# micahvista/VACmap

Hardware: AMD Instinct MI355X
Metric: aligned Gbp/s (whole node) + reads/s, 15 kb ONT-shape reads vs hg38-size ref, 1/2/4/8 MI355X (higher is better)
Workload: dtype i16/i32 DP + f64 chains

## Files before the change

### vacmap_amd/csrc/k_dp.hip

```cpp
#include "vmx_device.h"
#include "vmx_kernels.h"

__device__ __forceinline__ int vmx_tcode(uint8_t c) { return c < 4 ? (int)c : 6; }


__global__ void k_encode(const char* __restrict__ in, uint8_t* __restrict__ out, int64_t n) {
    int64_t i = (int64_t)blockIdx.x * blockDim.x + threadIdx.x;
    int64_t stride = (int64_t)gridDim.x * blockDim.x;
    for (; i < n; i += stride) out[i] = vmx_code((uint8_t)in[i]);
}

#define VMX_EXT_RING 512
__global__ void __launch_bounds__(64) k_extend(const uint8_t* __restrict__ tcodes, const int64_t* __restrict__ t_off,
                                               const uint8_t* __restrict__ qcodes, const int64_t* __restrict__ q_off, int n_prob,
                                               int match, int mismatch, int o, int e, int bw_in, int zdrop,
                                               int32_t* __restrict__ out_te, int32_t* __restrict__ out_qe, int32_t* __restrict__ out_sc, const int32_t* __restrict__ n_ptr) {
    if (n_ptr) n_prob = *n_ptr;
    __shared__ int sH[3][VMX_EXT_RING];
    __shared__ int sE[2][VMX_EXT_RING];
    __shared__ int sF[2][VMX_EXT_RING];
    const int lane = vmx_lane();
    const int RM = VMX_EXT_RING - 1;
    for (int p = blockIdx.x; p < n_prob; p += gridDim.x) {
        const uint8_t* T = tcodes + t_off[p];
// ... 331 lines not shown
                    const int j63 = t - 62;                                         \
                    if (j63 >= 1 && j63 <= ql && ((j63 & 63) == 0 || j63 == ql)) {                                    \
                        const int col = j63 - lane;                      \
                        if (col > ((j63 - 1) & ~63)) { bH[col] = sH; bE1[col] = sE1; bE2[col] = sE2; }                \
                    }                                                                                                 \
                }                                                                                                     \
            }
            for (int t0 = 0; t0 < W; t0 += 64) {
                const int jj = t0 + lane;
                int qchunk = jj < ql ? (int)Q[jj] : 4;
                int cH = 0, cE1 = VMX_NEG, cE2 = VMX_NEG;
                if (jj + 1 <= ql) {
                    if (s == 0) cH = vmx_gap_open_row(jj + 1, o1, e1, o2, e2);
                    else { cH = bH[jj + 1]; cE1 = bE1[jj + 1]; cE2 = bE2[jj + 1]; }
                }
                if (t0 >= 64 && t0 + 64 <= ql) {
                    for (int tt = 0; tt < 64; ++tt) { const int t = t0 + tt; VMX_GF_STEP(true) }
                } else {
                    int tend = W - t0; if (tend > 64) tend = 64;
                    for (int tt = 0; tt < tend; ++tt) { const int t = t0 + tt; const int j = t - lane + 1; VMX_GF_STEP(j >= 1 && j <= ql) }
                }
            }
#undef VMX_GF_STEP
            __syncthreads();
        }
        if (!trivial && !pk && lane == ((tl - 1) & 63)) out_score[p] = outH;
        int32_t sink = 0;
        if (pk) vmx_gapfill_fill16(T, Q, tl, ql, match, mismatch, o1, e1, o2, e2, tb, bH, SCORE ? &out_score[p] : &sink, lane);
}

template <bool SCORE>
__device__ __forceinline__ void vmx_gapfill_fill_body(const uint8_t* __restrict__ tcodes, const uint8_t* __restrict__ qcodes,
                                                     const vmx_dp_prob* __restrict__ probs, int n_prob, int match, int mismatch,
                                                     int o1, int e1, int o2, int e2, uint8_t* __restrict__ tb_pool,
                                                     int32_t* __restrict__ bnd_pool, int32_t* __restrict__ out_score,
                                                     const int32_t* __restrict__ order, int32_t* __restrict__ counter,
                                                     int32_t* __restrict__ redo_list = nullptr, int32_t* __restrict__ redo_cnt = nullptr, int redo_pass = 0,
                                                     uint8_t* __restrict__ redo_pool = nullptr) {
    const int lane = vmx_lane();
    int static_next = 4 * (int)blockIdx.x;
    if (redo_pass) {
        n_prob = redo_cnt[0]; order = redo_list; counter = redo_cnt + 1;
        while (true) {
            int q; { int v = 0; if (lane == 0) v = atomicAdd(redo_cnt + 2, 1); q = vmx_bcast0(v); }
            if (q >= n_prob) break;
            const int p = order[q];
            const int tl = probs[p].tl, ql = probs[p].ql;
            if (VMX_REDO_PK(tl, ql)) vmx_gapfill_fill_one<SCORE>(tcodes, qcodes, probs, p, match, mismatch, o1, e1, o2, e2, tb_pool, bnd_pool, out_score, lane, VMX_PK_FLAG, redo_pool);
        }
    }
    while (true) {
        int q0;
        if (order) { int v = 0; if (lane == 0) v = atomicAdd(counter, 4); q0 = vmx_bcast0(v); }
        else { q0 = static_next; static_next += 4 * (int)gridDim.x; }
        if (q0 >= n_prob) break;
        const int qg = q0 + (lane >> 4);
        const int pg = qg < n_prob ? (order ? order[qg] : qg) : -1;
        bool x4 = false, skip = false;
        {
            vmx_dp_prob pr; pr.tl = 0; pr.ql = 0; pr.t_off = 0; pr.q_off = 0; pr.tb_off = 0; pr.bnd_off = 0;
            if (pg >= 0) pr = probs[pg];
            skip = redo_pass && pg >= 0 && VMX_REDO_PK(pr.tl, pr.ql);
            x4 = pg >= 0 && !skip && pr.tl > 0 && pr.ql > 0 && VMX_DP16X4_OK(pr.tl, pr.ql);
            if (!SCORE && x4 && (lane & 15) == 0) out_score[pg] = 0;
            if (__any(x4))
                vmx_gapfill_fill16x4<SCORE>(tcodes + pr.t_off, qcodes + pr.q_off, x4 ? pr.tl : 0, x4 ? pr.ql : 0, match, mismatch, o1, e1, o2, e2, vmx_tb_ptr(tb_pool, redo_pool, pr.tb_off),
                                            bnd_pool + pr.bnd_off, &out_score[pg < 0 ? 0 : pg], lane);
        }
        for (int gk = 0; gk < 4; ++gk) {
            const int p = vmx_readlane(pg, 16 * gk);
            if (p < 0 || vmx_readlane((int)(x4 || skip), 16 * gk)) continue;
            vmx_gapfill_fill_one<SCORE>(tcodes, qcodes, probs, p, match, mismatch, o1, e1, o2, e2, tb_pool, bnd_pool, out_score, lane, 0, redo_pool);
        }
    }
}

__device__ __forceinline__ void vmx_gapfill_ad_pass(const uint8_t* __restrict__ tcodes, const uint8_t* __restrict__ qcodes, vmx_dp_prob* __restrict__ probs, int n_prob,
                                                   int match, int mismatch, int o1, int e1, int o2, int e2, uint8_t* __restrict__ tb_pool, int32_t* __restrict__ bnd_pool,
                                                   int32_t* __restrict__ out_score, const int32_t* __restrict__ order, const int32_t* __restrict__ range, int32_t* __restrict__ counter,
                                                   int32_t* __restrict__ redo_list, int32_t* __restrict__ redo_cnt, int ad_pct, unsigned long long* __restrict__ redo_bytes,
                                                   unsigned long long redo_cap, int tb_by_ns) {
    const int lane = vmx_lane();
    const int pct = ad_pct & 0xffff, pct_min = (ad_pct >> 16) & 0xffff;
    const int n_head = range[0] < n_prob ? range[0] : n_prob;
    bool head = n_head > 0;
    while (true) {
        int pX = -1, pY = -1;
        if (head) {
            int q; { int v = 0; if (lane == 0) v = atomicAdd(counter + 1, 1); q = vmx_bcast0(v); }
            if (q >= n_head) { head = false; continue; }
            if (lane < 16) pX = order[q];
        } else {
            int q0; { int v = 0; if (lane == 0) v = atomicAdd(counter, 8); q0 = n_head + vmx_bcast0(v); }
            if (q0 >= n_prob) break;
            const int qX = q0 + 2 * (lane >> 4), qY = qX + 1;
            if (qX < n_prob) pX = order[qX];
            if (qY < n_prob) pY = order[qY];
        }
        vmx_dp_prob prX, prY;
        prX.tl = 0; prX.ql = 0; prX.t_off = 0; prX.q_off = 0; prX.tb_off = 0; prY = prX;
        if (pX >= 0) prX = probs[pX];
        if (pY >= 0) prY = probs[pY];
        const bool x4X = pX >= 0 && prX.tl > 0 && prX.ql > 0 && VMX_DP16X4_OK(prX.tl, prX.ql), x4Y = pY >= 0 && prY.tl > 0 && prY.ql > 0 && VMX_DP16X4_OK(prY.tl, prY.ql);
        const int nsX = x4X ? vmx_ad_ns(prX.tl, prX.ql, match, o1, e1, o2, e2, pct, pct_min) : 0, nsY = x4Y ? vmx_ad_ns(prY.tl, prY.ql, match, o1, e1, o2, e2, pct, pct_min) : 0;
        const int ns = vmx_uniform_i32(vmx_wave_max_i32(nsX > nsY ? nsX : nsY));
        bool keepX = false, keepY = false, triedX = false, triedY = false;
        if (ns > 0) {
            int dloX = 0, dloY = 0;
            const bool fitX = !tb_by_ns || VMX_AD_W(nsX) == VMX_AD_W(ns), fitY = !tb_by_ns || VMX_AD_W(nsY) == VMX_AD_W(ns);
            const int gX = (nsX > 0 && fitX) ? vmx_ad_geom(prX.tl, prX.ql, ns, &dloX) : 0, gY = (nsY > 0 && fitY) ? vmx_ad_geom(prY.tl, prY.ql, ns, &dloY) : 0;
            const int tlX = gX > 0 ? prX.tl : 0, qlX = gX > 0 ? prX.ql : 0, tlY = gY > 0 ? prY.tl : 0, qlY = gY > 0 ? prY.ql : 0;
            int scX = 0, scY = 0;
#define VMX_AD_RUN(NSV) vmx_gapfill_fill_ad<NSV>(tcodes + prX.t_off, qcodes + prX.q_off, tlX, qlX, dloX, tb_pool + prX.tb_off, tcodes + prY.t_off, qcodes + prY.q_off, tlY, qlY, dloY, \
                                                 tb_pool + prY.tb_off, match, mismatch, o1, e1, o2, e2, lane, scX, scY)
            if (ns == 1) VMX_AD_RUN(1); else if (ns == 2) VMX_AD_RUN(2); else if (ns == 3) VMX_AD_RUN(3); else VMX_AD_RUN(4);
#undef VMX_AD_RUN
            triedX = gX > 0; triedY = gY > 0;
            keepX = gX > 0 && vmx_ad_proven(scX, prX.tl, prX.ql, gX, match, o1, e1, o2, e2);
            keepY = gY > 0 && vmx_ad_proven(scY, prY.tl, prY.ql, gY, match, o1, e1, o2, e2);
        }
        if ((lane & 15) == 0) {
            if (x4X) {
                out_score[pX] = keepX ? VMX_AD_FLAG + ns : 0;
                if (!keepX) {
                    if (triedX) atomicAdd(redo_cnt + 3, 1);
                    const unsigned long long need = (unsigned long long)VMX_REDO_TB_BYTES(prX.tl, prX.ql), at = atomicAdd(redo_bytes, need);
                    if (at + need > redo_cap) { probs[pX].tl = 0; probs[pX].ql = 0; probs[pX].tb_off = 0; }
                    else { probs[pX].tb_off = -(int64_t)at - 1; redo_list[atomicAdd(redo_cnt, 1)] = pX; }
                }
            }
            if (x4Y) {
                out_score[pY] = keepY ? VMX_AD_FLAG + ns : 0;
                if (!keepY) {
                    if (triedY) atomicAdd(redo_cnt + 3, 1);
                    const unsigned long long need = (unsigned long long)VMX_REDO_TB_BYTES(prY.tl, prY.ql), at = atomicAdd(redo_bytes, need);
                    if (at + need > redo_cap) { probs[pY].tl = 0; probs[pY].ql = 0; probs[pY].tb_off = 0; }
                    else { probs[pY].tb_off = -(int64_t)at - 1; redo_list[atomicAdd(redo_cnt, 1)] = pY; }
                }
            }
        }
        for (int gk = 0; gk < 8; ++gk) {
            const int p = vmx_readlane((gk & 1) ? pY : pX, 16 * (gk >> 1));
            if (p < 0 || vmx_readlane((int)((gk & 1) ? x4Y : x4X), 16 * (gk >> 1))) continue;
            vmx_gapfill_fill_one<false>(tcodes, qcodes, probs, p, match, mismatch, o1, e1, o2, e2, tb_pool, bnd_pool, out_score, lane);
        }
    }
}

__global__ void __launch_bounds__(64) k_gapfill_fill(const uint8_t* __restrict__ tcodes, const uint8_t* __restrict__ qcodes,
                                                     const vmx_dp_prob* __restrict__ probs, int n_prob, int match, int mismatch,
                                                     int o1, int e1, int o2, int e2, uint8_t* __restrict__ tb_pool,
                                                     int32_t* __restrict__ bnd_pool, int32_t* __restrict__ out_score,
                                                     const int32_t* __restrict__ order, int32_t* __restrict__ counter) {
    vmx_gapfill_fill_body<true>(tcodes, qcodes, probs, n_prob, match, mismatch, o1, e1, o2, e2, tb_pool, bnd_pool, out_score, order, counter);
}
__global__ void __launch_bounds__(64, 4) k_gapfill_fill_ns(const uint8_t* __restrict__ tcodes, const uint8_t* __restrict__ qcodes,
                                                        vmx_dp_prob* __restrict__ probs, int n_prob, int match, int mismatch,
                                                        int o1, int e1, int o2, int e2, uint8_t* __restrict__ tb_pool,
                                                        int32_t* __restrict__ bnd_pool, int32_t* __restrict__ out_score,
                                                        const int32_t* __restrict__ order, const int32_t* __restrict__ range, int32_t* __restrict__ counter,
                                                        int32_t* __restrict__ redo_list, int32_t* __restrict__ redo_cnt, int redo_pass, int ad_pct,
                                                        uint8_t* __restrict__ redo_pool, unsigned long long* __restrict__ redo_bytes, const int32_t* __restrict__ n_ptr,
                                                        unsigned long long redo_cap, int tb_by_ns) {
    if (n_ptr) n_prob = *n_ptr;
    if (redo_pass) vmx_gapfill_fill_body<false>(tcodes, qcodes, probs, n_prob, match, mismatch, o1, e1, o2, e2, tb_pool, bnd_pool, out_score, order, counter, redo_list, redo_cnt, 1, redo_pool);
    else vmx_gapfill_ad_pass(tcodes, qcodes, probs, n_prob, match, mismatch, o1, e1, o2, e2, tb_pool, bnd_pool, out_score, order, range, counter, redo_list, redo_cnt, ad_pct, redo_bytes, redo_cap, tb_by_ns);
}

__global__ void k_gapfill_trace(const uint8_t* __restrict__ tcodes, const uint8_t* __restrict__ qcodes,
                                const vmx_dp_prob* __restrict__ probs, int n_prob, int eqx, const uint8_t* __restrict__ tb_pool,
                                uint32_t* __restrict__ run_pool, char* __restrict__ cig_pool, int32_t* __restrict__ cig_len,
                                const int32_t* __restrict__ band_flag, const uint8_t* __restrict__ redo_pool, int spread, int32_t* __restrict__ cig_q,
                                const int32_t* __restrict__ n_ptr) {
    VMX_SETPRIO(3);
    if (n_ptr) n_prob = *n_ptr;
    const int gt = (int)(blockIdx.x * blockDim.x + threadIdx.x);
    if (spread > 1 && gt % spread) return;
    int p = spread > 1 ? gt / spread : gt;
    if (p >= n_prob) return;
    const vmx_dp_prob pr = probs[p];
    const uint8_t* T = tcodes + pr.t_off;
    const uint8_t* Q = qcodes + pr.q_off;
    const int tl = pr.tl, ql = pr.ql;
    const uint8_t* tb = vmx_tb_ptr(tb_pool, redo_pool, pr.tb_off);
    uint32_t* runs = run_pool + pr.run_off;
    char* cig = cig_pool + pr.cig_off;
    bool x4 = tl > 0 && ql > 0 && VMX_DP16X4_OK(tl, ql);
// ... 75 lines not shown
```

### vacmap_amd/csrc/vmx_device.h

```cpp
#ifndef VMX_DEVICE_H
#define VMX_DEVICE_H
#ifdef VMX_EMU
#include "hip_emu.h"
#define VMX_DYN_SHARED(type, name) type* name = (type*)hipemu::cur()->dynshared
#else
#include <hip/hip_runtime.h>
#define VMX_DYN_SHARED(type, name) extern __shared__ __attribute__((aligned(16))) type name[]
#endif
#include <stdint.h>

#define VMX_WAVE 64
#define VMX_NEG (-(1 << 28))
#define VMX_NOPRE (-9999999)

__device__ __forceinline__ int vmx_lane() { return (int)(threadIdx.x & 63); }

#ifdef VMX_EMU
__device__ __forceinline__ int vmx_shr1(int v) { return __shfl_up(v, 1); }
__device__ __forceinline__ int vmx_readlane(int v, int l) { return __shfl(v, l); }
#define VMX_SPIN_PAUSE() hipemu::yield()
#define VMX_CLOCK() 0LL
#else
__device__ __forceinline__ int vmx_shr1(int v) { return __builtin_amdgcn_update_dpp(v, v, 0x138, 0xf, 0xf, false); }
__device__ __forceinline__ int vmx_readlane(int v, int l) { return __builtin_amdgcn_readlane(v, l); }
#define VMX_SPIN_PAUSE() __builtin_amdgcn_s_sleep(1)
#define VMX_CLOCK() ((long long)wall_clock64())
#endif
#ifdef VMX_EMU
__device__ __forceinline__ int vmx_shr1_in(int v, int in) { int e = __shfl_up(v, 1); return vmx_lane() == 0 ? in : e; }
__device__ __forceinline__ int vmx_rol1(int v) { return __shfl(v, (vmx_lane() + 1) & 63); }
__device__ __forceinline__ int vmx_ror1(int v) { return __shfl(v, (vmx_lane() + 63) & 63); }
#else
__device__ __forceinline__ int vmx_shr1_in(int v, int in) { return __builtin_amdgcn_update_dpp(in, v, 0x138, 0xf, 0xf, false); }
__device__ __forceinline__ int vmx_rol1(int v) { return __builtin_amdgcn_update_dpp(v, v, 0x134, 0xf, 0xf, false); }
__device__ __forceinline__ int vmx_ror1(int v) { return __builtin_amdgcn_update_dpp(v, v, 0x13C, 0xf, 0xf, false); }
#endif
#ifdef VMX_EMU
__device__ __forceinline__ unsigned vmx_pk(int lo, int hi) { return ((unsigned)lo & 0xffffu) | ((unsigned)hi << 16); }
__device__ __forceinline__ int vmx_pk_lo(unsigned a) { return (int)(short)(a & 0xffffu); }
__device__ __forceinline__ int vmx_pk_hi(unsigned a) { return (int)(short)(a >> 16); }
__device__ __forceinline__ unsigned vmx_pk_add(unsigned a, unsigned b) { return vmx_pk(vmx_pk_lo(a) + vmx_pk_lo(b), vmx_pk_hi(a) + vmx_pk_hi(b)); }
__device__ __forceinline__ unsigned vmx_pk_sub(unsigned a, unsigned b) { return vmx_pk(vmx_pk_lo(a) - vmx_pk_lo(b), vmx_pk_hi(a) - vmx_pk_hi(b)); }
__device__ __forceinline__ unsigned vmx_pk_max(unsigned a, unsigned b) {
    const int l = vmx_pk_lo(a) > vmx_pk_lo(b) ? vmx_pk_lo(a) : vmx_pk_lo(b), h = vmx_pk_hi(a) > vmx_pk_hi(b) ? vmx_pk_hi(a) : vmx_pk_hi(b);
    return vmx_pk(l, h);
}
__device__ __forceinline__ unsigned vmx_pk_neg(unsigned a) { return (vmx_pk_lo(a) < 0 ? 0xffffu : 0u) | (vmx_pk_hi(a) < 0 ? 0xffff0000u : 0u); }
__device__ __forceinline__ unsigned vmx_pk_min_u16(unsigned a, unsigned b) { const unsigned al = a & 0xffffu, bl = b & 0xffffu, ah = a >> 16, bh = b >> 16; return (al < bl ? al : bl) | ((ah < bh ? ah : bh) << 16); }
__device__ __forceinline__ unsigned vmx_pk_mad(unsigned a, unsigned b, unsigned c) { return vmx_pk(vmx_pk_lo(a) * vmx_pk_lo(b) + vmx_pk_lo(c), vmx_pk_hi(a) * vmx_pk_hi(b) + vmx_pk_hi(c)); }
__device__ __forceinline__ unsigned vmx_alignbit16(unsigned hi, unsigned lo) { return (hi << 16) | (lo >> 16); }
#else
typedef short vmx_v2s __attribute__((ext_vector_type(2)));
__device__ __forceinline__ unsigned vmx_pk(int lo, int hi) { return ((unsigned)lo & 0xffffu) | ((unsigned)hi << 16); }
__device__ __forceinline__ int vmx_pk_lo(unsigned a) { return (int)(short)(a & 0xffffu); }
__device__ __forceinline__ int vmx_pk_hi(unsigned a) { return (int)(short)(a >> 16); }
__device__ __forceinline__ unsigned vmx_pk_add(unsigned a, unsigned b) { return __builtin_bit_cast(unsigned, (vmx_v2s)(__builtin_bit_cast(vmx_v2s, a) + __builtin_bit_cast(vmx_v2s, b))); }
__device__ __forceinline__ unsigned vmx_pk_sub(unsigned a, unsigned b) { return __builtin_bit_cast(unsigned, (vmx_v2s)(__builtin_bit_cast(vmx_v2s, a) - __builtin_bit_cast(vmx_v2s, b))); }
__device__ __forceinline__ unsigned vmx_pk_max(unsigned a, unsigned b) { return __builtin_bit_cast(unsigned, __builtin_elementwise_max(__builtin_bit_cast(vmx_v2s, a), __builtin_bit_cast(vmx_v2s, b))); }
__device__ __forceinline__ unsigned vmx_pk_neg(unsigned a) { unsigned r; asm("v_pk_ashrrev_i16 %0, 15, %1 op_sel_hi:[0,1]" : "=v"(r) : "v"(a)); return r; }
__device__ __forceinline__ unsigned vmx_pk_min_u16(unsigned a, unsigned b) { unsigned r; asm("v_pk_min_u16 %0, %1, %2" : "=v"(r) : "v"(a), "v"(b)); return r; }
__device__ __forceinline__ unsigned vmx_pk_mad(unsigned a, unsigned b, unsigned c) { unsigned r; asm("v_pk_mad_i16 %0, %1, %2, %3" : "=v"(r) : "v"(a), "v"(b), "v"(c)); return r; }
__device__ __forceinline__ unsigned vmx_alignbit16(unsigned hi, unsigned lo) { return __builtin_amdgcn_alignbit(hi, lo, 16); }
#endif
#ifdef VMX_EMU
__device__ __forceinline__ unsigned vmx_pk_bytes(unsigned b) { return (b & 0xffu) | ((b >> 8) & 0xff00u); }
#else
__device__ __forceinline__ unsigned vmx_pk_bytes(unsigned b) { return __builtin_amdgcn_perm(b, b, 0x0c0c0200u); }
#endif
#if defined(VMX_EMU) || defined(VMX_NOPRIO)
#define VMX_SETPRIO(p) ((void)0)
#else
#define VMX_SETPRIO(p) __builtin_amdgcn_s_setprio(p)
#endif
#ifdef VMX_EMU
__device__ __forceinline__ void vmx_wave_lds_fence() { __syncthreads(); }
#else
__device__ __forceinline__ void vmx_wave_lds_fence() { asm volatile("" ::: "memory"); }
#endif
__device__ __forceinline__ unsigned vmx_bfi(unsigned m, unsigned a, unsigned b) { return (m & a) | (~m & b); }
#ifdef VMX_EMU
__device__ __forceinline__ int vmx_uniform_i32(int v) { return v; }
#else
__device__ __forceinline__ int vmx_uniform_i32(int v) { return __builtin_amdgcn_readfirstlane(v); }
#endif
__device__ __forceinline__ long long vmx_uniform_i64(long long v) {
    union { long long d; int i[2]; } u; u.d = v;
    u.i[0] = vmx_uniform_i32(u.i[0]); u.i[1] = vmx_uniform_i32(u.i[1]);
    return u.d;
}
__device__ __forceinline__ double vmx_uniform_f64(double v) {
    union { double d; int i[2]; } u; u.d = v;
    u.i[0] = vmx_uniform_i32(u.i[0]); u.i[1] = vmx_uniform_i32(u.i[1]);
    return u.d;
}
#ifdef VMX_EMU
#define VMX_GLOBAL_PTR(T, p) (p)
#else
#define VMX_GLOBAL_PTR(T, p) ((T*)(__attribute__((address_space(1))) T*)(unsigned long long)vmx_uniform_i64((long long)(p)))
#endif
#ifdef VMX_EMU
__device__ __forceinline__ int vmx_bcast0(int v) { return __shfl(v, 0); }
#else
__device__ __forceinline__ int vmx_bcast0(int v) { return __builtin_amdgcn_readfirstlane(v); }
#endif
__device__ __forceinline__ double vmx_shr1_f64(double v) {
    union { double d; int i[2]; } u; u.d = v;
    u.i[0] = vmx_shr1(u.i[0]); u.i[1] = vmx_shr1(u.i[1]);
    return u.d;
}
__device__ __forceinline__ long long vmx_shr1_i64(long long v) {
    union { long long d; int i[2]; } u; u.d = v;
    u.i[0] = vmx_shr1(u.i[0]); u.i[1] = vmx_shr1(u.i[1]);
    return u.d;
}
struct vmx_cwin { int j, q, ls; double S; long long r; };
__device__ __forceinline__ void vmx_cwin_insert(vmx_cwin& w, int at, int k, double Sk, int qk, int lsk, long long rk, int lane) {
    const int sj = vmx_shr1(w.j), sq = vmx_shr1(w.q), sls = vmx_shr1(w.ls);
    const double sS = vmx_shr1_f64(w.S); const long long sr = vmx_shr1_i64(w.r);
    if (lane > at) { w.j = sj; w.q = sq; w.ls = sls; w.S = sS; w.r = sr; }
    else if (lane == at) { w.j = k; w.q = qk; w.ls = lsk; w.S = Sk; w.r = rk; }
}
__device__ __forceinline__ double vmx_readlane_f64(double v, int l) {
    union { double d; int i[2]; } u; u.d = v;
    u.i[0] = vmx_readlane(u.i[0], l); u.i[1] = vmx_readlane(u.i[1], l);
    return u.d;
}

__device__ __forceinline__ int vmx_wave_max_i32(int v) {
    for (int o = 32; o > 0; o >>= 1) { int x = __shfl_xor(v, o); v = x > v ? x : v; }
    return v;
}
__device__ __forceinline__ int vmx_wave_sum_i32(int v) {
    for (int o = 32; o > 0; o >>= 1) v += __shfl_xor(v, o);
    return v;
}
__device__ __forceinline__ long long vmx_wave_sum_i64(long long v) {
    for (int o = 32; o > 0; o >>= 1) v += __shfl_xor(v, o);
    return v;
}
__device__ __forceinline__ int vmx_wave_incl_scan_i32(int v) {
    int lane = vmx_lane();
    for (int o = 1; o < 64; o <<= 1) { int x = __shfl_up(v, o); if (lane >= o) v += x; }
    return v;
// ... 350 lines not shown
```

### vacmap_amd/csrc/vmx_dp_ad.h

```cpp
#ifndef VMX_DP_AD_H
#define VMX_DP_AD_H

#ifdef VMX_EMU
__device__ __forceinline__ int vmx_r16_shl1_in(int v, int in) { const int l = vmx_lane(); const int e = __shfl(v, (l & 48) | ((l + 1) & 15)); return (l & 15) == 15 ? in : e; }
__device__ __forceinline__ unsigned vmx_perm(unsigned s0, unsigned s1, unsigned sel) {
    unsigned r = 0;
    for (int b = 0; b < 4; ++b) {
        const unsigned c = (sel >> (8 * b)) & 0xffu;
        const unsigned v = c < 4 ? (s1 >> (8 * c)) & 0xffu : c < 8 ? (s0 >> (8 * (c - 4))) & 0xffu : 0u;
        r |= v << (8 * b);
    }
    return r;
}
#else
__device__ __forceinline__ int vmx_r16_shl1_in(int v, int in) { return __builtin_amdgcn_update_dpp(in, v, 0x101, 0xf, 0xf, false); }
__device__ __forceinline__ unsigned vmx_perm(unsigned s0, unsigned s1, unsigned sel) { return __builtin_amdgcn_perm(s0, s1, sel); }
#endif

#define VMX_AD_BIAS 8192
#define VMX_AD_NEGINF (-4096)
struct vmx_ad_consts { unsigned O1, O2, E1, E2, MATCH, NMIS, ONE, NEGP; };

__device__ __forceinline__ unsigned vmx_ad_cell(const vmx_ad_consts& K, unsigned upH, unsigned upE1, unsigned upE2, unsigned leftH, unsigned leftF1,
                                                unsigned leftF2, unsigned tc, unsigned qc, unsigned& H, unsigned& E1, unsigned& E2, unsigned& F1, unsigned& F2) {
    const unsigned a1 = upH - K.O1, a2 = upH - K.O2;
    unsigned b = (unsigned)((int)vmx_pk_sub(a1, upE1) >> 12) & 0x00080008u;
    b |= (unsigned)((int)vmx_pk_sub(a2, upE2) >> 11) & 0x00100010u;
    const unsigned e1v = vmx_pk_max(a1, upE1) - K.E1, e2v = vmx_pk_max(a2, upE2) - K.E2;
    const unsigned c1 = leftH - K.O1, c2 = leftH - K.O2;
    b |= (unsigned)((int)vmx_pk_sub(c1, leftF1) >> 10) & 0x00200020u;
    b |= (unsigned)((int)vmx_pk_sub(c2, leftF2) >> 9) & 0x00400040u;
    const unsigned f1v = vmx_pk_max(c1, leftF1) - K.E1, f2v = vmx_pk_max(c2, leftF2) - K.E2;
    unsigned h = vmx_pk_mad(vmx_pk_min_u16(tc ^ qc, K.ONE), K.NMIS, H) + K.MATCH;
    unsigned src = 0, m;
    m = vmx_pk_neg(vmx_pk_sub(h, e1v)); src = vmx_bfi(m, 0x00010001u, src); h = vmx_pk_max(h, e1v);
    m = vmx_pk_neg(vmx_pk_sub(h, f1v)); src = vmx_bfi(m, 0x00030003u, src); h = vmx_pk_max(h, f1v);
    m = vmx_pk_neg(vmx_pk_sub(h, e2v)); src = vmx_bfi(m, 0x00020002u, src); h = vmx_pk_max(h, e2v);
    m = vmx_pk_neg(vmx_pk_sub(h, f2v)); src = vmx_bfi(m, 0x00040004u, src); h = vmx_pk_max(h, f2v);
    H = h; E1 = e1v; E2 = e2v; F1 = f1v; F2 = f2v;
    return b | src;
}

template <int NS>
__device__ __forceinline__ unsigned vmx_ad_pick(const unsigned (&v)[NS], int k) {
    unsigned r = 0;
#pragma unroll
    for (int i = 0; i < NS; ++i) r |= v[i] & (unsigned)-(int)(k == i);
    return r;
}

template <int NS>
__device__ __forceinline__ void vmx_gapfill_fill_ad(const uint8_t* __restrict__ TX, const uint8_t* __restrict__ QX, int tlX, int qlX, int dloX, uint8_t* __restrict__ tbX,
                                                   const uint8_t* __restrict__ TY, const uint8_t* __restrict__ QY, int tlY, int qlY, int dloY, uint8_t* __restrict__ tbY,
                                                   int match, int mismatch, int o1, int e1, int o2, int e2, int lane, int& scoreX, int& scoreY) {
    const int l = lane & 15;
    vmx_ad_consts K;
    K.O1 = vmx_pk(o1, o1); K.O2 = vmx_pk(o2, o2); K.E1 = vmx_pk(e1, e1); K.E2 = vmx_pk(e2, e2);
    K.MATCH = vmx_pk(match, match); K.NMIS = vmx_pk(mismatch - match, mismatch - match); K.ONE = vmx_pk(1, 1); K.NEGP = vmx_pk(VMX_AD_NEGINF + VMX_AD_BIAS, VMX_AD_NEGINF + VMX_AD_BIAS);
    const int afX = (tlX > 0 && qlX > 0) ? tlX + qlX : 0, afY = (tlY > 0 && qlY > 0) ? tlY + qlY : 0;
    const int total = vmx_uniform_i32(vmx_wave_max_i32(afX > afY ? afX : afY));
    const int npairs = (total + 1) >> 1;
    const int poX = (afX + 1) >> 1, peX = afX >> 1, poY = (afY + 1) >> 1, peY = afY >> 1;
    const int hX = dloX >> 1, hY = dloY >> 1;
    auto tcf = [&](const uint8_t* T, int tl, int i) -> int { return (i >= 1 && i <= tl) ? vmx_tcode(T[i - 1]) : 5; };
    auto qcf = [&](const uint8_t* Q, int ql, int j) -> int { return (j >= 1 && j <= ql) ? (int)Q[j - 1] : 4; };
    unsigned tcode[NS], qcode[NS];
#pragma unroll
    for (int k = 0; k < NS; ++k) {
        tcode[k] = vmx_pk(tcf(TX, tlX, -hX - NS * l - k), tcf(TY, tlY, -hY - NS * l - k));
        qcode[k] = vmx_pk(qcf(QX, qlX, hX + NS * l + k), qcf(QY, qlY, hY + NS * l + k));
    }
    unsigned HA[NS], E1A[NS], E2A[NS], F1A[NS], F2A[NS], HC[NS], E1C[NS], E2C[NS], F1C[NS], F2C[NS];
    {
        const int l0X = (-dloX) / (2 * NS), k0X = ((-dloX) % (2 * NS)) >> 1, l0Y = (-dloY) / (2 * NS), k0Y = ((-dloY) % (2 * NS)) >> 1;
#pragma unroll
        for (int k = 0; k < NS; ++k) {
            const unsigned m = ((l == l0X && k == k0X) ? 0xffffu : 0u) | ((l == l0Y && k == k0Y) ? 0xffff0000u : 0u);
            HA[k] = vmx_bfi(m, vmx_pk(VMX_AD_BIAS, VMX_AD_BIAS), K.NEGP);
            E1A[k] = K.NEGP; E2A[k] = K.NEGP; F1A[k] = K.NEGP; F2A[k] = K.NEGP;
            HC[k] = K.NEGP; E1C[k] = K.NEGP; E2C[k] = K.NEGP; F1C[k] = K.NEGP; F2C[k] = K.NEGP;
        }
    }
    const int xfX = (qlX - tlX) - dloX, xfY = (qlY - tlY) - dloY;
    const int lfX = xfX / (2 * NS), kfX = (xfX % (2 * NS)) >> 1, lfY = xfY / (2 * NS), kfY = (xfY % (2 * NS)) >> 1;
    int finX = 0, finY = 0;
    constexpr int W = VMX_AD_W(NS);
    uint8_t* const pX = tbX + VMX_AD_TB_OFF_W(0, l, W);
    uint8_t* const pY = tbY + VMX_AD_TB_OFF_W(0, l, W);
    auto put = [&](uint8_t* at, unsigned w01, unsigned w23, bool hi) {
        if constexpr (W == 1) *at = (uint8_t)(hi ? (w01 >> 16) : w01);
        else if constexpr (W == 2) *(uint16_t*)at = (uint16_t)(hi ? (w01 >> 16) : w01);
        else *(uint32_t*)at = vmx_perm(w23, w01, hi ? 0x07060302u : 0x05040100u);
    };
    auto load_chunks = [&](int b16, unsigned& tch, unsigned& qch) {
        tch = vmx_pk(tcf(TX, tlX, b16 + 1 + l - hX), tcf(TY, tlY, b16 + 1 + l - hY));
        qch = vmx_pk(qcf(QX, qlX, b16 + 15 - l + hX + 16 * NS), qcf(QY, qlY, b16 + 15 - l + hY + 16 * NS));
    };
    unsigned tch, qch, ntch, nqch;
    load_chunks(0, ntch, nqch);
    for (int p0 = 0; p0 < npairs; p0 += 16) {
        tch = ntch; qch = nqch;
        load_chunks(p0 + 16, ntch, nqch);
        int pend = npairs - p0; if (pend > 16) pend = 16;
        for (int pp = 0; pp < pend; ++pp) {
            const int p = p0 + pp + 1;
            {
                const unsigned in = (unsigned)vmx_r16_shl1_in((int)qcode[0], (int)qch);
#pragma unroll
                for (int k = 0; k + 1 < NS; ++k) qcode[k] = qcode[k + 1];
                qcode[NS - 1] = in;
                qch = (unsigned)vmx_r16_ror1((int)qch);
            }
            unsigned bb[NS];
            {
                const unsigned nH = (unsigned)vmx_r16_shl1_in((int)HA[0], (int)K.NEGP), nE1 = (unsigned)vmx_r16_shl1_in((int)E1A[0], (int)K.NEGP),
                               nE2 = (unsigned)vmx_r16_shl1_in((int)E2A[0], (int)K.NEGP);
#pragma unroll
                for (int k = 0; k < NS; ++k) {
                    const unsigned uH = k + 1 < NS ? HA[k + 1 < NS ? k + 1 : 0] : nH, uE1 = k + 1 < NS ? E1A[k + 1 < NS ? k + 1 : 0] : nE1, uE2 = k + 1 < NS ? E2A[k + 1 < NS ? k + 1 : 0] : nE2;
                    bb[k] = vmx_ad_cell(K, uH, uE1, uE2, HA[k], F1A[k], F2A[k], tcode[k], qcode[k], HC[k], E1C[k], E2C[k], F1C[k], F2C[k]);
                }
            }
            {
                unsigned w01 = bb[0], w23 = 0;
                if (NS > 1) w01 |= bb[NS > 1 ? 1 : 0] << 8;
                if (NS > 2) w23 = bb[NS > 2 ? 2 : 0];
                if (NS > 3) w23 |= bb[NS > 3 ? 3 : 0] << 8;
                const size_t so = VMX_AD_TB_OFF_W(2 * p - 2, 0, W);
                if (p <= poX) put(pX + so, w01, w23, false);
                if (p <= poY) put(pY + so, w01, w23, true);
            }
            {
                const unsigned in = (unsigned)vmx_r16_shr1_in((int)tcode[NS - 1], (int)tch);
#pragma unroll
                for (int k = NS - 1; k > 0; --k) tcode[k] = tcode[k - 1];
                tcode[0] = in;
                tch = (unsigned)vmx_r16_rol1((int)tch);
            }
            {
                const unsigned nH = (unsigned)vmx_r16_shr1_in((int)HC[NS - 1], (int)K.NEGP), nF1 = (unsigned)vmx_r16_shr1_in((int)F1C[NS - 1], (int)K.NEGP),
                               nF2 = (unsigned)vmx_r16_shr1_in((int)F2C[NS - 1], (int)K.NEGP);
#pragma unroll
                for (int k = 0; k < NS; ++k) {
                    const unsigned lH = k > 0 ? HC[k > 0 ? k - 1 : 0] : nH, lF1 = k > 0 ? F1C[k > 0 ? k - 1 : 0] : nF1, lF2 = k > 0 ? F2C[k > 0 ? k - 1 : 0] : nF2;
                    bb[k] = vmx_ad_cell(K, HC[k], E1C[k], E2C[k], lH, lF1, lF2, tcode[k], qcode[k], HA[k], E1A[k], E2A[k], F1A[k], F2A[k]);
                }
            }
            {
                unsigned w01 = bb[0], w23 = 0;
                if (NS > 1) w01 |= bb[NS > 1 ? 1 : 0] << 8;
                if (NS > 2) w23 = bb[NS > 2 ? 2 : 0];
                if (NS > 3) w23 |= bb[NS > 3 ? 3 : 0] << 8;
                const size_t so = VMX_AD_TB_OFF_W(2 * p - 1, 0, W);
                if (p <= peX) put(pX + so, w01, w23, false);
                if (p <= peY) put(pY + so, w01, w23, true);
            }
            if (__any(p == poX || p == poY)) {
                const unsigned aX = vmx_ad_pick<NS>(HA, kfX), cX = vmx_ad_pick<NS>(HC, kfX), aY = vmx_ad_pick<NS>(HA, kfY), cY = vmx_ad_pick<NS>(HC, kfY);
                const unsigned vX = (afX & 1) ? cX : aX, vY = (afY & 1) ? cY : aY;
                if (p == poX && l == lfX) finX = vmx_pk_lo(vX) - VMX_AD_BIAS;
                if (p == poY && l == lfY) finY = vmx_pk_hi(vY) - VMX_AD_BIAS;
            }
        }
    }
    scoreX = __shfl(finX, (lane & 48) | (lfX & 15));
    scoreY = __shfl(finY, (lane & 48) | (lfY & 15));
}

__device__ __forceinline__ bool vmx_ad_proven(int score, int tl, int ql, int g, int match, int o1, int e1, int o2, int e2) {
    const int mn = tl < ql ? tl : ql;
    if (g < 1) return false;
    if (g > mn) return true;
    const long long U = (long long)match * mn - vmx_ad_margin(g, match, o1, e1, o2, e2);
    return (long long)score > U;
}
#endif
```

Baseline: 3.168.

## Tag traceback source in low bits of scaled unsigned 16-bit DP scores

Reworks the anti-diagonal 16x4 gap-fill cell so scores are scaled by 8 and biased into unsigned 16-bit lanes, with the low 3 bits carrying a source tag. The max operations then yield the traceback source directly, replacing the per-cell compare/negate/bfi chain. Traceback bytes are packed once per pair of cells via byte permutes. The aim is fewer VALU instructions per cell in the hot DP loop. In exchange it narrows the usable score range, so a host/device check now disables the AD path for scoring schemes that do not fit.

Measured after the change: 3.375, median of 6. 1.07x the previous value.

```diff
diff --git a/vacmap_amd/csrc/k_dp.hip b/vacmap_amd/csrc/k_dp.hip
--- a/vacmap_amd/csrc/k_dp.hip
+++ b/vacmap_amd/csrc/k_dp.hip
@@ -437,6 +437,7 @@
                                                    unsigned long long redo_cap, int tb_by_ns) {
     const int lane = vmx_lane();
     const int pct = ad_pct & 0xffff, pct_min = (ad_pct >> 16) & 0xffff;
+    const bool ad_ok = vmx_ad_scores_ok(match, mismatch, o1, e1, o2, e2);
     const int n_head = range[0] < n_prob ? range[0] : n_prob;
     bool head = n_head > 0;
     while (true) {
@@ -457,7 +458,7 @@
         if (pX >= 0) prX = probs[pX];
         if (pY >= 0) prY = probs[pY];
         const bool x4X = pX >= 0 && prX.tl > 0 && prX.ql > 0 && VMX_DP16X4_OK(prX.tl, prX.ql), x4Y = pY >= 0 && prY.tl > 0 && prY.ql > 0 && VMX_DP16X4_OK(prY.tl, prY.ql);
-        const int nsX = x4X ? vmx_ad_ns(prX.tl, prX.ql, match, o1, e1, o2, e2, pct, pct_min) : 0, nsY = x4Y ? vmx_ad_ns(prY.tl, prY.ql, match, o1, e1, o2, e2, pct, pct_min) : 0;
+        const int nsX = x4X && ad_ok ? vmx_ad_ns(prX.tl, prX.ql, match, o1, e1, o2, e2, pct, pct_min) : 0, nsY = x4Y && ad_ok ? vmx_ad_ns(prY.tl, prY.ql, match, o1, e1, o2, e2, pct, pct_min) : 0;
         const int ns = vmx_uniform_i32(vmx_wave_max_i32(nsX > nsY ? nsX : nsY));
         bool keepX = false, keepY = false, triedX = false, triedY = false;
         if (ns > 0) {
diff --git a/vacmap_amd/csrc/vmx_device.h b/vacmap_amd/csrc/vmx_device.h
--- a/vacmap_amd/csrc/vmx_device.h
+++ b/vacmap_amd/csrc/vmx_device.h
@@ -47,6 +47,7 @@
 }
 __device__ __forceinline__ unsigned vmx_pk_neg(unsigned a) { return (vmx_pk_lo(a) < 0 ? 0xffffu : 0u) | (vmx_pk_hi(a) < 0 ? 0xffff0000u : 0u); }
 __device__ __forceinline__ unsigned vmx_pk_min_u16(unsigned a, unsigned b) { const unsigned al = a & 0xffffu, bl = b & 0xffffu, ah = a >> 16, bh = b >> 16; return (al < bl ? al : bl) | ((ah < bh ? ah : bh) << 16); }
+__device__ __forceinline__ unsigned vmx_pk_max_u16(unsigned a, unsigned b) { const unsigned al = a & 0xffffu, bl = b & 0xffffu, ah = a >> 16, bh = b >> 16; return (al > bl ? al : bl) | ((ah > bh ? ah : bh) << 16); }
 __device__ __forceinline__ unsigned vmx_pk_mad(unsigned a, unsigned b, unsigned c) { return vmx_pk(vmx_pk_lo(a) * vmx_pk_lo(b) + vmx_pk_lo(c), vmx_pk_hi(a) * vmx_pk_hi(b) + vmx_pk_hi(c)); }
 __device__ __forceinline__ unsigned vmx_alignbit16(unsigned hi, unsigned lo) { return (hi << 16) | (lo >> 16); }
 #else
@@ -59,6 +60,8 @@
 __device__ __forceinline__ unsigned vmx_pk_max(unsigned a, unsigned b) { return __builtin_bit_cast(unsigned, __builtin_elementwise_max(__builtin_bit_cast(vmx_v2s, a), __builtin_bit_cast(vmx_v2s, b))); }
 __device__ __forceinline__ unsigned vmx_pk_neg(unsigned a) { unsigned r; asm("v_pk_ashrrev_i16 %0, 15, %1 op_sel_hi:[0,1]" : "=v"(r) : "v"(a)); return r; }
 __device__ __forceinline__ unsigned vmx_pk_min_u16(unsigned a, unsigned b) { unsigned r; asm("v_pk_min_u16 %0, %1, %2" : "=v"(r) : "v"(a), "v"(b)); return r; }
+typedef unsigned short vmx_v2u __attribute__((ext_vector_type(2)));
+__device__ __forceinline__ unsigned vmx_pk_max_u16(unsigned a, unsigned b) { return __builtin_bit_cast(unsigned, __builtin_elementwise_max(__builtin_bit_cast(vmx_v2u, a), __builtin_bit_cast(vmx_v2u, b))); }
 __device__ __forceinline__ unsigned vmx_pk_mad(unsigned a, unsigned b, unsigned c) { unsigned r; asm("v_pk_mad_i16 %0, %1, %2, %3" : "=v"(r) : "v"(a), "v"(b), "v"(c)); return r; }
 __device__ __forceinline__ unsigned vmx_alignbit16(unsigned hi, unsigned lo) { return __builtin_amdgcn_alignbit(hi, lo, 16); }
 #endif
diff --git a/vacmap_amd/csrc/vmx_dp_ad.h b/vacmap_amd/csrc/vmx_dp_ad.h
--- a/vacmap_amd/csrc/vmx_dp_ad.h
+++ b/vacmap_amd/csrc/vmx_dp_ad.h
@@ -17,28 +17,56 @@
 __device__ __forceinline__ unsigned vmx_perm(unsigned s0, unsigned s1, unsigned sel) { return __builtin_amdgcn_perm(s0, s1, sel); }
 #endif
 
-#define VMX_AD_BIAS 8192
 #define VMX_AD_NEGINF (-4096)
-struct vmx_ad_consts { unsigned O1, O2, E1, E2, MATCH, NMIS, ONE, NEGP; };
-
-__device__ __forceinline__ unsigned vmx_ad_cell(const vmx_ad_consts& K, unsigned upH, unsigned upE1, unsigned upE2, unsigned leftH, unsigned leftF1,
-                                                unsigned leftF2, unsigned tc, unsigned qc, unsigned& H, unsigned& E1, unsigned& E2, unsigned& F1, unsigned& F2) {
-    const unsigned a1 = upH - K.O1, a2 = upH - K.O2;
-    unsigned b = (unsigned)((int)vmx_pk_sub(a1, upE1) >> 12) & 0x00080008u;
-    b |= (unsigned)((int)vmx_pk_sub(a2, upE2) >> 11) & 0x00100010u;
-    const unsigned e1v = vmx_pk_max(a1, upE1) - K.E1, e2v = vmx_pk_max(a2, upE2) - K.E2;
-    const unsigned c1 = leftH - K.O1, c2 = leftH - K.O2;
-    b |= (unsigned)((int)vmx_pk_sub(c1, leftF1) >> 10) & 0x00200020u;
-    b |= (unsigned)((int)vmx_pk_sub(c2, leftF2) >> 9) & 0x00400040u;
-    const unsigned f1v = vmx_pk_max(c1, leftF1) - K.E1, f2v = vmx_pk_max(c2, leftF2) - K.E2;
-    unsigned h = vmx_pk_mad(vmx_pk_min_u16(tc ^ qc, K.ONE), K.NMIS, H) + K.MATCH;
-    unsigned src = 0, m;
-    m = vmx_pk_neg(vmx_pk_sub(h, e1v)); src = vmx_bfi(m, 0x00010001u, src); h = vmx_pk_max(h, e1v);
-    m = vmx_pk_neg(vmx_pk_sub(h, f1v)); src = vmx_bfi(m, 0x00030003u, src); h = vmx_pk_max(h, f1v);
-    m = vmx_pk_neg(vmx_pk_sub(h, e2v)); src = vmx_bfi(m, 0x00020002u, src); h = vmx_pk_max(h, e2v);
-    m = vmx_pk_neg(vmx_pk_sub(h, f2v)); src = vmx_bfi(m, 0x00040004u, src); h = vmx_pk_max(h, f2v);
-    H = h; E1 = e1v; E2 = e2v; F1 = f1v; F2 = f2v;
-    return b | src;
+#define VMX_AD_CSH 12
+#define VMX_AD_TE1 6u
+#define VMX_AD_TF1 3u
+#define VMX_AD_TE2 1u
+#define VMX_AD_TF2 0u
+__host__ __device__ constexpr long long vmx_ad_imax(long long a, long long b) { return a > b ? a : b; }
+__host__ __device__ constexpr long long vmx_ad_imin(long long a, long long b) { return a < b ? a : b; }
+__host__ __device__ constexpr long long vmx_ad_bias(int mismatch, int o1, int e1, int o2, int e2) {
+    return -((long long)VMX_AD_NEGINF - (long long)(VMX_DP16X4_MAX + 1) * vmx_ad_imax(e1, e2) - vmx_ad_imax(vmx_ad_imax(o1, o2), -(long long)mismatch));
+}
+__host__ __device__ constexpr bool vmx_ad_scores_ok(int match, int mismatch, int o1, int e1, int o2, int e2) {
+    return match >= 0 && mismatch <= match && 8LL * (match - mismatch) <= (1 << VMX_AD_CSH) && o1 >= 0 && e1 >= 0 && o2 >= 0 && e2 >= 0 &&
+           (long long)match * (VMX_DP16X4_MAX / 2 + 1) + vmx_ad_bias(mismatch, o1, e1, o2, e2) <= 8191 &&
+           vmx_ad_imin(mismatch, 0) * (VMX_DP16X4_MAX / 2) - vmx_ad_imin(o1 + (long long)e1 * VMX_DP16X4_MAX, o2 + (long long)e2 * VMX_DP16X4_MAX)
+               - vmx_ad_imax(o1, o2) - vmx_ad_imax(e1, e2) > (long long)VMX_AD_NEGINF + vmx_ad_imax(o1, o2);
+}
+static_assert(vmx_ad_scores_ok(2, -4, 4, 2, 24, 1), "the gap fill's own scoring (vmx_align.hip: gf_score) must fit the tagged 16-bit domain");
+struct vmx_ad_consts { unsigned O1, O2, E1, E2, MATCH, PEN, NH, NE1, NE2, NF1, NF2; };
+
+__device__ __forceinline__ void vmx_ad_cell(const vmx_ad_consts& K, unsigned upH, unsigned upE1, unsigned upE2, unsigned leftH, unsigned leftF1,
+                                            unsigned leftF2, unsigned tc, unsigned qc, unsigned& H, unsigned& E1, unsigned& E2, unsigned& F1, unsigned& F2,
+                                            unsigned (&w)[5]) {
+    const unsigned e1v = vmx_pk_max_u16(upH - K.O1, upE1) - K.E1, e2v = vmx_pk_max_u16(upH - K.O2, upE2) - K.E2;
+    const unsigned f1v = vmx_pk_max_u16(leftH - K.O1, leftF1) - K.E1, f2v = vmx_pk_max_u16(leftH - K.O2, leftF2) - K.E2;
+    E1 = e1v & ~((7u ^ VMX_AD_TE1) * 0x00010001u); E2 = e2v & ~((7u ^ VMX_AD_TE2) * 0x00010001u);
+    F1 = f1v & ~((7u ^ VMX_AD_TF1) * 0x00010001u); F2 = f2v & ~((7u ^ VMX_AD_TF2) * 0x00010001u);
+    const unsigned hd = H + K.MATCH - vmx_pk_min_u16(tc ^ qc, K.PEN);
+    const unsigned h = vmx_pk_max_u16(vmx_pk_max_u16(hd, E1), vmx_pk_max_u16(vmx_pk_max_u16(F1, E2), F2));
+    H = h | 0x00070007u;
+    w[0] = h; w[1] = e1v; w[2] = e2v; w[3] = f1v; w[4] = f2v;
+}
+
+__device__ __forceinline__ unsigned vmx_ad_bytes(const unsigned (&a)[5], const unsigned (&b)[5]) {
+    constexpr unsigned SEL = 0x06020400u;
+    const unsigned gh = vmx_perm(b[0], a[0], SEL), ge1 = vmx_perm(b[1], a[1], SEL), ge2 = vmx_perm(b[2], a[2], SEL);
+    const unsigned gf1 = vmx_perm(b[3], a[3], SEL), gf2 = vmx_perm(b[4], a[4], SEL);
+    const unsigned src = vmx_perm(0x00010000u, 0x03000204u, gh & 0x07070707u);
+    unsigned op = vmx_bfi(0x01010101u, ge1, ge2);
+    op = vmx_bfi(0x04040404u, gf1, op);
+    op = vmx_bfi(0x08080808u, (gf2 << 3) | (gf2 >> 29), op);
+    return src | (((op & 0x0f0f0f0fu) ^ 0x0f0f0f0fu) << 3);
+}
+
+template <int NS>
+__device__ __forceinline__ void vmx_ad_pack(const unsigned (&w)[NS][5], unsigned& w01, unsigned& w23) {
+    w01 = vmx_ad_bytes(w[0], w[NS > 1 ? 1 : 0]);
+    w23 = 0;
+    if (NS > 2) w23 = vmx_ad_bytes(w[NS > 2 ? 2 : 0], w[NS > 3 ? 3 : 0]);
+    if (NS == 3) w23 &= 0x00ff00ffu;
 }
 
 template <int NS>
@@ -55,15 +83,19 @@
                                                    int match, int mismatch, int o1, int e1, int o2, int e2, int lane, int& scoreX, int& scoreY) {
     const int l = lane & 15;
     vmx_ad_consts K;
-    K.O1 = vmx_pk(o1, o1); K.O2 = vmx_pk(o2, o2); K.E1 = vmx_pk(e1, e1); K.E2 = vmx_pk(e2, e2);
-    K.MATCH = vmx_pk(match, match); K.NMIS = vmx_pk(mismatch - match, mismatch - match); K.ONE = vmx_pk(1, 1); K.NEGP = vmx_pk(VMX_AD_NEGINF + VMX_AD_BIAS, VMX_AD_NEGINF + VMX_AD_BIAS);
+    K.O1 = vmx_pk(8 * o1, 8 * o1); K.O2 = vmx_pk(8 * o2, 8 * o2); K.E1 = vmx_pk(8 * e1, 8 * e1); K.E2 = vmx_pk(8 * e2, 8 * e2);
+    K.MATCH = vmx_pk(8 * match, 8 * match); K.PEN = vmx_pk(8 * (match - mismatch), 8 * (match - mismatch));
+    const int bias = (int)vmx_ad_bias(mismatch, o1, e1, o2, e2);
+    const unsigned neg = 8u * (unsigned)(VMX_AD_NEGINF + bias);
+    K.NH = (neg + 7u) * 0x00010001u; K.NE1 = (neg + VMX_AD_TE1) * 0x00010001u; K.NE2 = (neg + VMX_AD_TE2) * 0x00010001u;
+    K.NF1 = (neg + VMX_AD_TF1) * 0x00010001u; K.NF2 = (neg + VMX_AD_TF2) * 0x00010001u;
     const int afX = (tlX > 0 && qlX > 0) ? tlX + qlX : 0, afY = (tlY > 0 && qlY > 0) ? tlY + qlY : 0;
     const int total = vmx_uniform_i32(vmx_wave_max_i32(afX > afY ? afX : afY));
     const int npairs = (total + 1) >> 1;
     const int poX = (afX + 1) >> 1, peX = afX >> 1, poY = (afY + 1) >> 1, peY = afY >> 1;
     const int hX = dloX >> 1, hY = dloY >> 1;
-    auto tcf = [&](const uint8_t* T, int tl, int i) -> int { return (i >= 1 && i <= tl) ? vmx_tcode(T[i - 1]) : 5; };
-    auto qcf = [&](const uint8_t* Q, int ql, int j) -> int { return (j >= 1 && j <= ql) ? (int)Q[j - 1] : 4; };
+    auto tcf = [&](const uint8_t* T, int tl, int i) -> int { return ((i >= 1 && i <= tl) ? vmx_tcode(T[i - 1]) : 5) << VMX_AD_CSH; };
+    auto qcf = [&](const uint8_t* Q, int ql, int j) -> int { return ((j >= 1 && j <= ql) ? (int)Q[j - 1] : 4) << VMX_AD_CSH; };
     unsigned tcode[NS], qcode[NS];
 #pragma unroll
     for (int k = 0; k < NS; ++k) {
@@ -76,9 +108,9 @@
 #pragma unroll
         for (int k = 0; k < NS; ++k) {
             const unsigned m = ((l == l0X && k == k0X) ? 0xffffu : 0u) | ((l == l0Y && k == k0Y) ? 0xffff0000u : 0u);
-            HA[k] = vmx_bfi(m, vmx_pk(VMX_AD_BIAS, VMX_AD_BIAS), K.NEGP);
-            E1A[k] = K.NEGP; E2A[k] = K.NEGP; F1A[k] = K.NEGP; F2A[k] = K.NEGP;
-            HC[k] = K.NEGP; E1C[k] = K.NEGP; E2C[k] = K.NEGP; F1C[k] = K.NEGP; F2C[k] = K.NEGP;
+            HA[k] = vmx_bfi(m, (8u * (unsigned)bias + 7u) * 0x00010001u, K.NH);
+            E1A[k] = K.NE1; E2A[k] = K.NE2; F1A[k] = K.NF1; F2A[k] = K.NF2;
+            HC[k] = K.NH; E1C[k] = K.NE1; E2C[k] = K.NE2; F1C[k] = K.NF1; F2C[k] = K.NF2;
         }
     }
     const int xfX = (qlX - tlX) - dloX, xfY = (qlY - tlY) - dloY;
@@ -111,21 +143,19 @@
                 qcode[NS - 1] = in;
                 qch = (unsigned)vmx_r16_ror1((int)qch);
             }
-            unsigned bb[NS];
-            {
-                const unsigned nH = (unsigned)vmx_r16_shl1_in((int)HA[0], (int)K.NEGP), nE1 = (unsigned)vmx_r16_shl1_in((int)E1A[0], (int)K.NEGP),
-                               nE2 = (unsigned)vmx_r16_shl1_in((int)E2A[0], (int)K.NEGP);
+            unsigned w[NS][5];
+            {
+                const unsigned nH = (unsigned)vmx_r16_shl1_in((int)HA[0], (int)K.NH), nE1 = (unsigned)vmx_r16_shl1_in((int)E1A[0], (int)K.NE1),
+                               nE2 = (unsigned)vmx_r16_shl1_in((int)E2A[0], (int)K.NE2);
 #pragma unroll
                 for (int k = 0; k < NS; ++k) {
                     const unsigned uH = k + 1 < NS ? HA[k + 1 < NS ? k + 1 : 0] : nH, uE1 = k + 1 < NS ? E1A[k + 1 < NS ? k + 1 : 0] : nE1, uE2 = k + 1 < NS ? E2A[k + 1 < NS ? k + 1 : 0] : nE2;
-                    bb[k] = vmx_ad_cell(K, uH, uE1, uE2, HA[k], F1A[k], F2A[k], tcode[k], qcode[k], HC[k], E1C[k], E2C[k], F1C[k], F2C[k]);
+                    vmx_ad_cell(K, uH, uE1, uE2, HA[k], F1A[k], F2A[k], tcode[k], qcode[k], HC[k], E1C[k], E2C[k], F1C[k], F2C[k], w[k]);
                 }
             }
             {
-                unsigned w01 = bb[0], w23 = 0;
-                if (NS > 1) w01 |= bb[NS > 1 ? 1 : 0] << 8;
-                if (NS > 2) w23 = bb[NS > 2 ? 2 : 0];
-                if (NS > 3) w23 |= bb[NS > 3 ? 3 : 0] << 8;
+                unsigned w01, w23;
+                vmx_ad_pack<NS>(w, w01, w23);
                 const size_t so = VMX_AD_TB_OFF_W(2 * p - 2, 0, W);
                 if (p <= poX) put(pX + so, w01, w23, false);
                 if (p <= poY) put(pY + so, w01, w23, true);
@@ -138,19 +168,17 @@
                 tch = (unsigned)vmx_r16_rol1((int)tch);
             }
             {
-                const unsigned nH = (unsigned)vmx_r16_shr1_in((int)HC[NS - 1], (int)K.NEGP), nF1 = (unsigned)vmx_r16_shr1_in((int)F1C[NS - 1], (int)K.NEGP),
-                               nF2 = (unsigned)vmx_r16_shr1_in((int)F2C[NS - 1], (int)K.NEGP);
+                const unsigned nH = (unsigned)vmx_r16_shr1_in((int)HC[NS - 1], (int)K.NH), nF1 = (unsigned)vmx_r16_shr1_in((int)F1C[NS - 1], (int)K.NF1),
+                               nF2 = (unsigned)vmx_r16_shr1_in((int)F2C[NS - 1], (int)K.NF2);
 #pragma unroll
                 for (int k = 0; k < NS; ++k) {
                     const unsigned lH = k > 0 ? HC[k > 0 ? k - 1 : 0] : nH, lF1 = k > 0 ? F1C[k > 0 ? k - 1 : 0] : nF1, lF2 = k > 0 ? F2C[k > 0 ? k - 1 : 0] : nF2;
-                    bb[k] = vmx_ad_cell(K, HC[k], E1C[k], E2C[k], lH, lF1, lF2, tcode[k], qcode[k], HA[k], E1A[k], E2A[k], F1A[k], F2A[k]);
+                    vmx_ad_cell(K, HC[k], E1C[k], E2C[k], lH, lF1, lF2, tcode[k], qcode[k], HA[k], E1A[k], E2A[k], F1A[k], F2A[k], w[k]);
                 }
             }
             {
-                unsigned w01 = bb[0], w23 = 0;
-                if (NS > 1) w01 |= bb[NS > 1 ? 1 : 0] << 8;
-                if (NS > 2) w23 = bb[NS > 2 ? 2 : 0];
-                if (NS > 3) w23 |= bb[NS > 3 ? 3 : 0] << 8;
+                unsigned w01, w23;
+                vmx_ad_pack<NS>(w, w01, w23);
                 const size_t so = VMX_AD_TB_OFF_W(2 * p - 1, 0, W);
                 if (p <= peX) put(pX + so, w01, w23, false);
                 if (p <= peY) put(pY + so, w01, w23, true);
@@ -158,8 +186,8 @@
             if (__any(p == poX || p == poY)) {
                 const unsigned aX = vmx_ad_pick<NS>(HA, kfX), cX = vmx_ad_pick<NS>(HC, kfX), aY = vmx_ad_pick<NS>(HA, kfY), cY = vmx_ad_pick<NS>(HC, kfY);
                 const unsigned vX = (afX & 1) ? cX : aX, vY = (afY & 1) ? cY : aY;
-                if (p == poX && l == lfX) finX = vmx_pk_lo(vX) - VMX_AD_BIAS;
-                if (p == poY && l == lfY) finY = vmx_pk_hi(vY) - VMX_AD_BIAS;
+                if (p == poX && l == lfX) finX = (int)((vX & 0xffffu) >> 3) - bias;
+                if (p == poY && l == lfY) finY = (int)(vY >> 19) - bias;
             }
         }
     }
```
